# hahnec/stofnet

Measured on AMD Instinct MI355X. Metric: RF waveforms/sec StofNet inference rf_scale=10, higher is better.
Workload: dtype f32 via split-fp16 x3 MFMA operands (hi+lo, fp32 accumulate), device-side exact-f32 re-run on fp16 range overflow; 1 GPU; C2 StofNet.forward [4096,1,2000] -> [4096,1,20000] per GPU, upsample_factor=10, SemiGlobalBlock on, seeded-random weights (seed 3008); rows_per_gpu=4096, L=2000, upsample_factor=10, precision=auto

## Files before the change

stofnet_amd/csrc/convstack.hip:

```cpp
#include <hip/hip_runtime.h>
#include <stdlib.h>
#include <type_traits>
#include "stof_common.h"
#include "stof_hip_util.h"

namespace stof {
int launch_conv_cl(const float* x, const float* w, const float* bias, const float* residual, const float* saved, float* y,
                   int64_t N, int64_t L, int32_t cin, int32_t cout, int32_t K, int32_t act, int32_t precision,
                   int32_t period, int32_t valid_len, hipStream_t stream, const int* run_if);
}

using namespace stof;

typedef float floatx16 __attribute__((ext_vector_type(16)));
typedef _Float16 half8 __attribute__((ext_vector_type(8)));
typedef _Float16 half4 __attribute__((ext_vector_type(4)));

namespace {

constexpr int LAG_LAST = 34;
constexpr int SGB_NW = 2;
constexpr int SGB_WAVES_PER_SIMD = (SGB_NW <= 2) ? 2 : 1;
constexpr int ROWB = ROWF * 4;

// ... 868 lines not shown
                else tail(std::false_type{});
                STAMP_ADD(5);
                __syncthreads();
                STAMP_ADD(2);
                continue;
            }
            auto last_chunks = [&]() {
#pragma unroll
                for (int cc = 0; cc < BODY_CHUNKS_LAST; cc += 2) { do_chunk(wf[0], bf0, bf1, cc); do_chunk(wf[1], bf1, bf0, cc + 1); }
            };
            last_chunks();
            STAMP_ADD(4);

            {
                bool valid[NT];
                int tt[NT], nn[NT];
#pragma unroll
                for (int k = 0; k < NT; ++k) {
                    const int off = 32 * (NT * ni + k) + ln;
                    const int g = R0 + off;
                    decode_row(nR, tR, off, nn[k], tt[k]);
                    int nw, tw;
                    vmap(n0 + nn[k], tt[k], nw, tw);
                    valid[k] = (g >= 0) && (g < gend) && (tt[k] < L) && (tw >= 0) && (tw < Ltrue) &&
                               (tt[k] >= p.halo) && (tt[k] < p.halo + p.seg_len);
                    nn[k] = nw - n0;
                    tt[k] = tw;
                }
                if (p.status != nullptr) {
                    bool bad = false;
#pragma unroll
                    for (int k = 0; k < NT; ++k)
#pragma unroll
                        for (int e = 0; e < 16; ++e) bad = bad || !(fabsf(acc[k][e]) <= 3.0e38f);
                    if (__any(bad) && lane == 0) atomicOr(p.status, 1);
                }
#pragma unroll
                for (int k = 0; k < NT; ++k) {
                    if (!valid[k]) continue;
                    float* const orow = p.y + ((size_t)(n0 + nn[k]) * Ltrue + tt[k]) * r;
#pragma unroll
                    for (int gg = 0; gg < 4; ++gg) {
                        const int c0 = 32 * mi + 8 * gg + 4 * lh;
                        if (c0 >= r) continue;
                        const float vv[4] = {acc[k][4 * gg], acc[k][4 * gg + 1], acc[k][4 * gg + 2], acc[k][4 * gg + 3]};
                        if ((r & 3) == 0) {
                            st4(orow + c0, make_float4(vv[0], vv[1], vv[2], vv[3]));
                        } else {
#pragma unroll
                            for (int e = 0; e < 4; ++e)
                                if (c0 + e < r) orow[c0 + e] = vv[e];
                        }
                    }
                }
            }
            STAMP_ADD(5);
            __syncthreads();
            STAMP_ADD(2);
            }
        }
    }
#ifdef STOF_STAMPS
    if (lane == 0 && p.stamps) {
        unsigned long long* o = p.stamps + ((size_t)blockIdx.x * 4 + wave) * 8;
        for (int i = 0; i < 6; ++i) o[i] = tsum[i];
        o[6] = stamp() - tstart;
        o[7] = (unsigned long long)nsteps;
    }
#endif
}

constexpr int BODY_P2_C1F = 640;
#include "body_p2.h"

struct SgbParams {
    const float* x;
    float* pooled;
    const float* c1;
    const float* cbias;
    const float* chunks;
    int N, L, P, tiles_per_wf;
    const int* run_if;
    unsigned char* arg;
};

template <int PREC, int NW, bool ARG = false>
__global__ __launch_bounds__(256, SGB_WAVES_PER_SIMD) void sgb_contract_pool_kernel(const SgbParams p) {
    constexpr int SHAPE = PREC == STOF_PREC_F16X3 ? 16 : 32;
    static_assert(!ARG || PREC == STOF_PREC_F16X3, "the arg-max output lives in the split-fp16 form");
    static_assert(NW % 2 == 0, "80*NW must be a multiple of 32");
    constexpr int ROWS = SGB_SCALE * NW;
    constexpr int MT = ROWS / 32;
    constexpr int TR = ROWS + 4;
    constexpr int RAWN = TR + 8;
    constexpr int RF = SHAPE == 16 ? ROWF16 : ROWF;
    constexpr int ROWB = RF * 4;
    extern __shared__ __attribute__((aligned(16))) float smem[];
    char* const act = reinterpret_cast<char*>(smem);
    float* const raw = smem + TR * RF;

    const int tid = threadIdx.x;
    const int lane = tid & 63, wave = tid >> 6;
    const int ln = lane & 31, lh = lane >> 5;
    const int n = blockIdx.x / p.tiles_per_wf;
    const int w0 = (blockIdx.x - n * p.tiles_per_wf) * NW;
    const int L = p.L;
    const int tbase = SGB_SCALE * w0 - 2;
    if (p.run_if != nullptr && *p.run_if == 0) return;

    const uint4* const wbase = reinterpret_cast<const uint4*>(p.chunks) + wave * 64 + lane;
    auto wload = [&](int c, int f) -> uint4 { return wbase[((size_t)c * FRAGS_PER_CHUNK + f) * 256]; };
    uint4 wf[2][FRAGS_PER_CHUNK];
#pragma unroll
    for (int f = 0; f < FRAGS_PER_CHUNK; ++f) {
        wf[0][f] = wload(0, f);
        wf[1][f] = wload(1, f);
    }

    for (int i = tid; i < RAWN; i += 256) {
        const int t = tbase - 4 + i;
        raw[i] = (t >= 0 && t < L) ? p.x[(size_t)n * L + t] : 0.f;
    }
    __syncthreads();
    {
        const int cq = tid & 15, rl = tid >> 4;
        float w1[4][9], b1[4];
#pragma unroll
        for (int i = 0; i < 4; ++i) {
#pragma unroll
            for (int d = 0; d < 9; ++d) w1[i][d] = p.c1[(4 * cq + i) * 10 + d];
            b1[i] = p.c1[(4 * cq + i) * 10 + 9];
        }
        for (int row = rl; row < TR; row += 16) {
            const int t = tbase + row;
            float v[4];
#pragma unroll
            for (int i = 0; i < 4; ++i) {
                float a = b1[i];
#pragma unroll
                for (int d = 0; d < 9; ++d) a = fmaf(w1[i][d], raw[row + d], a);
                v[i] = fmaxf(a, 0.f);
            }
            const bool valid = (t >= 0) && (t < L);
            store_act4<PREC>(act + row * ROWB, 4 * cq,
                             valid ? make_float4(v[0], v[1], v[2], v[3]) : make_float4(0.f, 0.f, 0.f, 0.f));
        }
    }
    __syncthreads();

    int c = 0;
    if constexpr (SHAPE == 16) {
        constexpr int MW = SGB_SCALE / 16;
        const int j16 = lane & 15, q4 = lane >> 4;
        for (int ocb = 0; ocb < 4; ++ocb) {
            floatx4 acc[NW][MW][2];
#pragma unroll
            for (int w = 0; w < NW; ++w)
#pragma unroll
                for (int m = 0; m < MW; ++m)
#pragma unroll
                    for (int nt = 0; nt < 2; ++nt)
#pragma unroll
                        for (int e = 0; e < 4; ++e) acc[w][m][nt][e] = 0.f;
            constexpr int NUNIT = 10 * NW;
            auto aload = [&](uint4 (&a)[MW][2], int uu) {
                const int cc = uu / NW, w = uu % NW;
                const int d = cc >> 1, hh = cc & 1;
                const char* arow = act + (SGB_SCALE * w + j16 + d) * ROWB + 64 * hh + 16 * q4;
#pragma unroll
                for (int m = 0; m < MW; ++m) {
                    a[m][0] = ldq(arow + 16 * m * ROWB);
                    a[m][1] = ldq(arow + 16 * m * ROWB + 128);
                }
            };
            auto mfma16 = [](const uint4& a, const uint4& b, floatx4 cacc) {
                return __builtin_amdgcn_mfma_f32_16x16x32_f16(as_h8(a), as_h8(b), cacc, 0, 0, 0);
            };
            auto do_unit = [&](uint4 (&acur)[MW][2], uint4 (&anext)[MW][2], int uu) {
                const int cc = uu / NW, w = uu % NW;
                uint4 (&wq)[FRAGS_PER_CHUNK] = wf[cc & 1];
                const int c2 = (c + 2 < SGB_NCHUNK) ? c + 2 : 0;
                aload(anext, uu + 1 < NUNIT ? uu + 1 : 0);
#pragma unroll
                for (int m = 0; m < MW; ++m) {
                    acc[w][m][0] = mfma16(acur[m][0], wq[0], acc[w][m][0]);
                    acc[w][m][1] = mfma16(acur[m][0], wq[2], acc[w][m][1]);
                    acc[w][m][0] = mfma16(acur[m][1], wq[0], acc[w][m][0]);
                    acc[w][m][1] = mfma16(acur[m][1], wq[2], acc[w][m][1]);
                    acc[w][m][0] = mfma16(acur[m][0], wq[1], acc[w][m][0]);
                    acc[w][m][1] = mfma16(acur[m][0], wq[3], acc[w][m][1]);
                }
                if (w == NW - 1) {
#pragma unroll
                    for (int f = 0; f < FRAGS_PER_CHUNK; ++f) wq[f] = wload(c2, f);
                    ++c;
                }
#pragma unroll
                for (int i = 0; i < MW * 2; ++i) {
                    __builtin_amdgcn_sched_group_barrier(0x008, 3, 0);
                    __builtin_amdgcn_sched_group_barrier(0x100, 1, 0);
                }
                if (w == NW - 1) __builtin_amdgcn_sched_group_barrier(0x020, FRAGS_PER_CHUNK, 0);
                __builtin_amdgcn_sched_barrier(0);
            };
            uint4 af0[MW][2], af1[MW][2];
            if (ocb == 0) aload(af0, 0);
            static_assert(NUNIT % 2 == 0, "units alternate between two fragment sets");
#pragma unroll
            for (int uu = 0; uu < NUNIT; uu += 2) {
                do_unit(af0, af1, uu);
                do_unit(af1, af0, uu + 1);
            }
#pragma unroll
            for (int nt = 0; nt < 2; ++nt) {
                const int oc = 128 * ocb + 32 * wave + 16 * nt + j16;
                const float bias = p.cbias[oc];
#pragma unroll
                for (int w = 0; w < NW; ++w) {
                    float mval = -INFINITY;
                    if constexpr (ARG) {
                        int bi = 0;
#pragma unroll
                        for (int m = 0; m < MW; ++m)
#pragma unroll
                            for (int e = 0; e < 4; ++e) {
                                const float v = acc[w][m][nt][e];
                                const bool up = v > mval;
                                mval = up ? v : mval;
                                bi = up ? 16 * m + 4 * q4 + e : bi;
                            }
#pragma unroll
                        for (int off = 16; off <= 32; off <<= 1) {
                            const float ov = __shfl_xor(mval, off);
                            const int oi = __shfl_xor(bi, off);
                            const bool take = (ov > mval) || (ov == mval && oi < bi);
                            mval = take ? ov : mval;
                            bi = take ? oi : bi;
                        }
                        if (q4 == 0 && w0 + w < p.P) p.arg[((size_t)n * p.P + w0 + w) * NF_SGB + oc] = (unsigned char)bi;
                    } else {
#pragma unroll
                        for (int m = 0; m < MW; ++m)
#pragma unroll
                            for (int e = 0; e < 4; ++e) mval = fmaxf(mval, acc[w][m][nt][e]);
                        mval = fmaxf(mval, __shfl_xor(mval, 16));
                        mval = fmaxf(mval, __shfl_xor(mval, 32));
                    }
                    mval += bias;
                    mval = mval > 0.f ? mval : 0.01f * mval;
                    if (q4 == 0 && w0 + w < p.P)
                        p.pooled[((size_t)n * p.P + w0 + w) * NF_SGB + oc] = mval;
                }
            }
        }
    } else {
    for (int ocb = 0; ocb < 4; ++ocb) {
        floatx16 acc[MT];
#pragma unroll
        for (int m = 0; m < MT; ++m)
#pragma unroll
            for (int e = 0; e < 16; ++e) acc[m][e] = 0.f;

        constexpr int UPC = FRAGS_PER_CHUNK;
        constexpr int NUNIT = 10 * UPC;
        auto aload = [&](uint4 (&a)[MT], int uu) {
            const int cc = uu / UPC, sub = uu % UPC;
            const int d = cc >> 1, hh = cc & 1;
            const char* arow = act + (ln + d) * ROWB;
#pragma unroll
            for (int m = 0; m < MT; ++m) a[m] = ldq(arow + 32 * m * ROWB + act_frag_off(sub, hh, lh));
        };
        auto do_unit = [&](uint4 (&acur)[MT], uint4 (&anext)[MT], int uu) {
            const int cc = uu / UPC, sub = uu % UPC;
            uint4 (&w)[FRAGS_PER_CHUNK] = wf[cc & 1];
            const int c2 = (c + 2 < SGB_NCHUNK) ? c + 2 : 0;
            aload(anext, uu + 1 < NUNIT ? uu + 1 : 0);
#pragma unroll
            for (int m = 0; m < MT; ++m) acc[m] = mma_fp32(acur[m], w[sub], acc[m]);
            w[sub] = wload(c2, sub);
#pragma unroll
            for (int i = 0; i < MT; ++i) {
                __builtin_amdgcn_sched_group_barrier(0x008, 4, 0);
                __builtin_amdgcn_sched_group_barrier(0x100, 1, 0);
            }
            if (sub == UPC - 1) ++c;
            __builtin_amdgcn_sched_barrier(0);
        };
        uint4 af0[MT], af1[MT];
        if (ocb == 0) aload(af0, 0);
#pragma unroll
        for (int uu = 0; uu < NUNIT; uu += 2) {
            do_unit(af0, af1, uu);
            do_unit(af1, af0, uu + 1);
        }
        const int oc = 128 * ocb + 32 * wave + ln;
        const float bias = p.cbias[oc];
        float wmax[NW];
#pragma unroll
        for (int w = 0; w < NW; ++w) wmax[w] = -INFINITY;
#pragma unroll
        for (int m = 0; m < MT; ++m)
#pragma unroll
            for (int v = 0; v < 16; ++v) {
                const int w = (32 * m + 8 * (v >> 2)) / SGB_SCALE;
                wmax[w] = fmaxf(wmax[w], acc[m][v]);
            }
#pragma unroll
        for (int w = 0; w < NW; ++w) {
            float mval = fmaxf(wmax[w], __shfl_xor(wmax[w], 32));
            mval += bias;
            mval = mval > 0.f ? mval : 0.01f * mval;
            if (lh == 0 && w0 + w < p.P)
                p.pooled[((size_t)n * p.P + w0 + w) * NF_SGB + oc] = mval;
        }
    }
    }
}

__global__ __launch_bounds__(256) void onsets_finalize_kernel(const OnsetPartial* __restrict__ ws, int nslots, int nb, int r,
                                                              int half, int* __restrict__ counts, int* __restrict__ idx,
                                                              long long idx_cap) {
    const int lane = threadIdx.x & 63;
    const int row = blockIdx.x * 4 + (threadIdx.x >> 6);
    if (row >= nb) return;
    const OnsetPartial* e = ws + (size_t)row * nslots;
    float m = -INFINITY, lo = INFINITY;
    for (int s = lane; s < nslots; s += 64)
        if (e[s].written) { m = fmaxf(m, e[s].m); lo = fminf(lo, e[s].lo); }
#pragma unroll
    for (int o = 32; o > 0; o >>= 1) { m = fmaxf(m, __shfl_xor(m, o)); lo = fminf(lo, __shfl_xor(lo, o)); }
    const bool emit = (m > 0.f) || (m < 0.f && (lo == m || half == 0));
    int nout = 0;
    if (emit) {
        const unsigned long long lt_mask = (lane == 0) ? 0ull : (~0ull >> (64 - lane));
        int* out = idx + (long long)row * idx_cap;
        for (int s0 = 0; s0 < nslots; s0 += 64) {
            const int sl = s0 + lane;
            unsigned long long match = __ballot(sl < nslots && e[sl].written && e[sl].m == m);
            while (match) {
            const int s = s0 + __builtin_ctzll(match);
            match &= match - 1;
            const OnsetPartial p = e[s];
            for (int q0 = 0; q0 < 16 * r; q0 += 64) {
                const int q = q0 + lane, j = q / r, c = q - j * r;
                const bool hit = q < 16 * r && ((p.eq[c & 3] >> (j + 16 * (c >> 2))) & 1ull);
                const unsigned long long hm = __ballot(hit);
                if (hit) {
                    const long long pos = nout + __builtin_popcountll(hm & lt_mask);
                    if (pos < idx_cap) out[pos] = (p.tw_base + j) * r + c;
                }
                nout += __builtin_popcountll(hm);
            }
            }
        }
    }
    if (lane == 0) counts[row] = nout;
}

constexpr int BODY_S = 192, BODY_RING = 256, BODY_RAWRING = 256;
inline bool body_p2_rows_ok(int seg_len, int halo) { return seg_len + 2 * halo + GAP >= 2 * BODY_S; }
constexpr int ONSET_MAX_SEGS = 32;

constexpr int64_t onset_seg_slots(int64_t seg_len) { return seg_len / 16 + 2; }
constexpr int64_t onset_max_slots(int64_t L) { return L / 16 + 3 * ONSET_MAX_SEGS; }

struct OnsetArgs {
    OnsetPartial* ws;
    int32_t* counts;
    int32_t* idx;
    int64_t idx_cap;
    int half;
};
constexpr int64_t SUB_BATCH = 4096;

constexpr size_t sgb_lds_bytes(int rowf) {
    return (size_t)((SGB_SCALE * SGB_NW + 4) * rowf + SGB_SCALE * SGB_NW + 12) * sizeof(float);
}

template <int PREC>
int launch_forward(const stof_net_desc* desc, const void* packed_dev, const float* x, float* y, int64_t N,
                   int64_t L, void* workspace, hipStream_t stream, void* const* events, int32_t* status,
                   const int32_t* run_if, const OnsetArgs* onsets = nullptr) {
    const int force_nseg_log2 = desc->seg_policy > 0 ? desc->seg_policy - 1 : -1;
    const int r = desc->upsample_factor;
    const bool has_sgb = desc->semi_global_scale != 1;
    const int64_t P = L / SGB_SCALE;
    const int64_t rem = L - P * SGB_SCALE;

    const float* base = static_cast<const float*>(packed_dev);
    uint64_t off = sizeof(PackedHeader) / sizeof(float);
    const float* c1 = base + off;      off += 64 * 10;
    const float* bias = base + off;    off += 13 * 64;
    const float* body = base + off;    off += (uint64_t)BODY_NCHUNK * BODY_CHUNK_F;
    const float* last16 = nullptr;
    if (PREC == STOF_PREC_F16X3 && r <= 16) { last16 = base + off; off += LAST16_F; }
    const float* cbias = base + off;   off += NF_SGB;
    const float* cchunks = base + off; off += (uint64_t)SGB_NCHUNK * SGB_CHUNK_F;
    const float* ew = base + off;      off += 5ull * NF_SGB * NF;
    const float* ebias = base + off;

    static const bool body_p2 = PREC == STOF_PREC_F16X3 && body_p2_enabled();
    constexpr int RF = PREC == STOF_PREC_F16X3 ? ROWF16 : ROWF;
    using Lds = BodyLds<BODY_S, BODY_RING, BODY_RAWRING, RF>;
    const size_t body_p2_bytes = Lds::BYTES + BODY_P2_C1F * sizeof(float);
    const auto body_kernel = &body_sweep_kernel<PREC, BODY_S, BODY_RING, BODY_RAWRING>;
    const auto body_p2_kernel = &body_sweep_p2_kernel<BODY_S, BODY_RING, BODY_RAWRING>;
    const auto sgb_kernel = &sgb_contract_pool_kernel<PREC, SGB_NW>;
    const size_t sgb_bytes = sgb_lds_bytes(RF);
    static LdsLimitOnce body_lds, body_p2_lds, sgb_lds;
    if (int st = body_lds.ensure(reinterpret_cast<const void*>(body_kernel), (int)Lds::BYTES)) return st;
    if (body_p2)
        if (int st = body_p2_lds.ensure(reinterpret_cast<const void*>(body_p2_kernel), (int)body_p2_bytes)) return st;
    if (int st = sgb_lds.ensure(reinterpret_cast<const void*>(sgb_kernel), (int)sgb_bytes)) return st;
    const int ncu = device_cu_count();

    for (int64_t b0 = 0; b0 < N; b0 += SUB_BATCH) {
        const int64_t nb = (N - b0) < SUB_BATCH ? (N - b0) : SUB_BATCH;
        const float* xb = x + b0 * L;
        float* yb = y ? y + b0 * L * r : nullptr;
        float* pooled = nullptr;
        float* sgb = nullptr;
        const bool ev = events && b0 == 0;
        if (ev) (void)hipEventRecord(static_cast<hipEvent_t>(events[0]), stream);
        if (has_sgb && P > 0) {
            pooled = static_cast<float*>(workspace);
            sgb = pooled + nb * P * NF_SGB;
            SgbParams sp;
            sp.x = xb; sp.pooled = pooled; sp.c1 = c1; sp.cbias = cbias; sp.chunks = cchunks;
            sp.N = (int)nb; sp.L = (int)L; sp.P = (int)P;
            sp.tiles_per_wf = (int)((P + SGB_NW - 1) / SGB_NW);
            sp.run_if = run_if;
            sp.arg = nullptr;
            hipLaunchKernelGGL(sgb_kernel, dim3((unsigned)(nb * sp.tiles_per_wf)), dim3(256), sgb_bytes, stream, sp);
            if (ev) (void)hipEventRecord(static_cast<hipEvent_t>(events[1]), stream);
            {
                const int st = stof::launch_conv_cl(pooled, ew, ebias, nullptr, nullptr, sgb, 1, nb * (P + 2), NF_SGB, NF, 5,
                                                     2, PREC, (int)(P + 2), (int)P, stream, run_if);
                if (st != STOF_OK) return st;
            }
            if (ev) (void)hipEventRecord(static_cast<hipEvent_t>(events[2]), stream);
        } else if (ev) {
            (void)hipEventRecord(static_cast<hipEvent_t>(events[1]), stream);
            (void)hipEventRecord(static_cast<hipEvent_t>(events[2]), stream);
        }
        BodyParams bp;
        bp.x = xb; bp.sgb = (has_sgb && P > 0) ? sgb : nullptr; bp.y = yb;
        bp.c1 = c1; bp.bias = bias; bp.chunks = body; bp.last16 = last16;
        bp.N = (int)nb; bp.L = (int)L; bp.r = r; bp.P = (int)P; bp.rem_half = (int)(rem / 2);
        bp.stamps = nullptr;
        bp.dump = nullptr; bp.dump_stride = 0;
        bp.gin = nullptr; bp.fwd_dump = nullptr;
        bp.status = status;
        bp.run_if = run_if;
        bp.nseg_log2 = 0;
        {
            int64_t best = -1;
            for (int k = 0; k <= 5; ++k) {
                const int64_t ns = (int64_t)1 << k;
                if (k > 0 && L / ns < BODY_S / 2) break;
                const int64_t lv = (L + ns - 1) / ns + (k > 0 ? 76 : 0);
                const int64_t nvk = nb * ns;
                const int64_t w = nvk < ncu ? nvk : ncu;
                const int64_t per = (nvk + w - 1) / w;
                const int64_t steps = (per * (lv + GAP) - GAP + LAG_LAST + BODY_S - 1) / BODY_S;
                if (best < 0 || steps < best) { best = steps; bp.nseg_log2 = k; }
            }
        }
        int64_t nseg = (int64_t)1 << bp.nseg_log2;
        if (force_nseg_log2 >= 0) { bp.nseg_log2 = force_nseg_log2; nseg = (int64_t)1 << force_nseg_log2; }
        bp.seg_len = (int)((L + nseg - 1) / nseg);
        bp.halo = nseg > 1 ? 38 : 0;
        const int64_t nv = nb * nseg;
        bp.N = (int)nv;
        bp.onset_ws = nullptr; bp.onset_slots = 0; bp.onset_seg_slots = 0;
        if (onsets != nullptr) {
            bp.onset_seg_slots = (int)onset_seg_slots(bp.seg_len);
            bp.onset_slots = (int)(nseg * bp.onset_seg_slots);
            bp.onset_ws = onsets->ws;
            if (hipMemsetAsync(onsets->ws, 0, (size_t)nb * bp.onset_slots * sizeof(OnsetPartial), stream) != hipSuccess)
                return STOF_ERR_HIP;
        }
#ifdef STOF_STAMPS
        if (workspace) bp.stamps = reinterpret_cast<unsigned long long*>(static_cast<char*>(workspace) + (size_t)(nb * P * (NF_SGB + NF)) * sizeof(float) + 256);
#endif
        int64_t wgs = nv < ncu ? nv : ncu;
        bp.wf_per_wg = (int)((nv + wgs - 1) / wgs);
        wgs = (nv + bp.wf_per_wg - 1) / bp.wf_per_wg;
        if (body_p2 && body_p2_rows_ok(bp.seg_len, bp.halo))
            hipLaunchKernelGGL(body_p2_kernel, dim3((unsigned)wgs), dim3(256), body_p2_bytes, stream, bp);
        else
            hipLaunchKernelGGL(body_kernel, dim3((unsigned)wgs), dim3(256), Lds::BYTES, stream, bp);
        if (ev) (void)hipEventRecord(static_cast<hipEvent_t>(events[3]), stream);
        if (onsets != nullptr)
            hipLaunchKernelGGL(onsets_finalize_kernel, dim3((unsigned)((nb + 3) / 4)), dim3(256), 0, stream, onsets->ws,
                               bp.onset_slots, (int)nb, r, onsets->half, onsets->counts + b0, onsets->idx + b0 * onsets->idx_cap,
                               (long long)onsets->idx_cap);
    }
    if (hipGetLastError() != hipSuccess) return STOF_ERR_HIP;
    return STOF_OK;
}

int forward_impl(const stof_net_desc* desc, const void* packed_dev, const float* x, float* y, int64_t N, int64_t L,
                 void* workspace, size_t workspace_bytes, void* stream_, void* const* events, int32_t* status,
                 const int32_t* run_if = nullptr, const OnsetArgs* onsets = nullptr) {
    if (!desc || N < 0 || L < 0) return STOF_ERR_BAD_ARG;
    if (desc->precision != STOF_PREC_FP32 && desc->precision != STOF_PREC_F16X3) return STOF_ERR_UNSUPPORTED;
    if (desc->seg_policy < 0 || desc->seg_policy > 6) return STOF_ERR_UNSUPPORTED;
    const int r = desc->upsample_factor;
    if (r < 1 || r > 64) return STOF_ERR_UNSUPPORTED;
    const bool has_sgb = desc->semi_global_scale != 1;
    if (has_sgb && desc->semi_global_scale != SGB_SCALE) return STOF_ERR_UNSUPPORTED;
    const int64_t P = L / SGB_SCALE;
    if (has_sgb && L > 0 && P == 0) return STOF_ERR_POOL_EMPTY;
    if (has_sgb && ((L - P * SGB_SCALE) & 1)) return STOF_ERR_ODD_SGB_REMAINDER;
    if (N == 0 || L == 0) return STOF_OK;
    if (!packed_dev || !x || (!y && !onsets)) return STOF_ERR_BAD_ARG;
    if ((L + GAP) * SUB_BATCH > 0x7fffffffLL) return STOF_ERR_UNSUPPORTED;
    if (has_sgb && (!workspace || workspace_bytes < stof_forward_workspace_bytes(desc, N, L)))
        return STOF_ERR_WORKSPACE;
    hipStream_t stream = static_cast<hipStream_t>(stream_);
    if (desc->precision == STOF_PREC_FP32)
        return launch_forward<STOF_PREC_FP32>(desc, packed_dev, x, y, N, L, workspace, stream, events, status, run_if, onsets);
    return launch_forward<STOF_PREC_F16X3>(desc, packed_dev, x, y, N, L, workspace, stream, events, status, run_if, onsets);
}

}

extern "C" size_t stof_forward_workspace_bytes(const stof_net_desc* desc, int64_t N, int64_t L) {
    if (!desc || N <= 0 || L <= 0 || desc->semi_global_scale == 1) return 0;
    const int64_t nb = N < SUB_BATCH ? N : SUB_BATCH;
    const int64_t P = L / SGB_SCALE;
#ifdef STOF_STAMPS
    return (size_t)(nb * P * (NF_SGB + NF)) * sizeof(float) + 256 + 256 * 4 * 8 * 8 + 64;
#else
    return (size_t)(nb * P * (NF_SGB + NF)) * sizeof(float) + 256;
#endif
}

extern "C" int stof_forward(const stof_net_desc* desc, const void* packed_dev, const float* x, float* y,
                            int64_t N, int64_t L, void* workspace, size_t workspace_bytes, void* stream) {
    return forward_impl(desc, packed_dev, x, y, N, L, workspace, workspace_bytes, stream, nullptr, nullptr);
}

extern "C" int stof_forward_checked(const stof_net_desc* desc, const void* packed_dev, const float* x, float* y,
                                    int64_t N, int64_t L, void* workspace, size_t workspace_bytes, void* stream,
                                    int32_t* status_dev) {
    if (!status_dev) return STOF_ERR_BAD_ARG;
    return forward_impl(desc, packed_dev, x, y, N, L, workspace, workspace_bytes, stream, nullptr, status_dev);
}

extern "C" int stof_forward_events(const stof_net_desc* desc, const void* packed_dev, const float* x, float* y,
                                   int64_t N, int64_t L, void* workspace, size_t workspace_bytes, void* stream,
                                   void* const* events, int32_t* status_dev) {
    if (!events) return STOF_ERR_BAD_ARG;
    for (int e = 0; e < STOF_FORWARD_EVENTS; ++e)
        if (!events[e]) return STOF_ERR_BAD_ARG;
    return forward_impl(desc, packed_dev, x, y, N, L, workspace, workspace_bytes, stream, events, status_dev);
}

static size_t onsets_partials_offset(const stof_net_desc* desc, int64_t N, int64_t L) {
    return (stof_forward_workspace_bytes(desc, N, L) + 255) / 256 * 256;
}

extern "C" size_t stof_forward_onsets_workspace_bytes(const stof_net_desc* desc, int64_t N, int64_t L) {
    if (!desc || N <= 0 || L <= 0) return 0;
    const int64_t nb = N < SUB_BATCH ? N : SUB_BATCH;
    return onsets_partials_offset(desc, N, L) + (size_t)nb * onset_max_slots(L) * sizeof(OnsetPartial);
}

extern "C" int stof_forward_onsets(const stof_net_desc* desc, const void* packed_dev, const float* x, float* y, int64_t N,
                                   int64_t L, int32_t window_size, int32_t* counts, int32_t* idx, int64_t idx_cap,
                                   void* workspace, size_t workspace_bytes, void* stream, int32_t* status_dev) {
    if (!desc || !counts || (!idx && idx_cap > 0) || idx_cap < 0 || window_size < 0) return STOF_ERR_BAD_ARG;
    if (desc->precision != STOF_PREC_F16X3 || desc->upsample_factor > 16 || L < 32)
        return STOF_ERR_UNSUPPORTED;
    if (N > 0 && L > 0 && (!workspace || workspace_bytes < stof_forward_onsets_workspace_bytes(desc, N, L))) return STOF_ERR_WORKSPACE;
    OnsetArgs oa;
    oa.ws = reinterpret_cast<OnsetPartial*>(static_cast<char*>(workspace) + onsets_partials_offset(desc, N, L));
    oa.counts = counts; oa.idx = idx; oa.idx_cap = idx_cap;
    oa.half = (window_size / 2 * 2 + 1 - 1) / 2;
    return forward_impl(desc, packed_dev, x, y, N, L, workspace, workspace_bytes, stream, nullptr, status_dev, nullptr, &oa);
}

extern "C" int stof_forward_auto(const stof_net_desc* desc, const void* packed_f16x3_dev, const void* packed_fp32_dev,
                                 const float* x, float* y, int64_t N, int64_t L, void* workspace, size_t workspace_bytes,
                                 void* stream, int32_t* status_dev, void* const* events) {
    if (!desc || !status_dev) return STOF_ERR_BAD_ARG;
    if (events)
        for (int e = 0; e < STOF_FORWARD_EVENTS; ++e)
            if (!events[e]) return STOF_ERR_BAD_ARG;
    stof_net_desc d16 = *desc, d32 = *desc;
    d16.precision = STOF_PREC_F16X3;
    d32.precision = STOF_PREC_FP32;
    if (N > 0 && L > 0 && hipMemsetAsync(status_dev, 0, sizeof(int32_t), static_cast<hipStream_t>(stream)) != hipSuccess)
        return STOF_ERR_HIP;
    const int st = forward_impl(&d16, packed_f16x3_dev, x, y, N, L, workspace, workspace_bytes, stream, events, status_dev);
    if (st != STOF_OK) return st;
    return forward_impl(&d32, packed_fp32_dev, x, y, N, L, workspace, workspace_bytes, stream, nullptr, nullptr, status_dev);
}

namespace {

struct SweepPackArgs {
    const float* p[26];
    float* blob;
    int r;
};

__global__ __launch_bounds__(256) void sweep_pack_kernel(const SweepPackArgs a) {
    const long long i = blockIdx.x * 256ll + threadIdx.x;
    const long long n_c1 = 640, n_bias = 13 * 64, n_body = (long long)BODY_NCHUNK * BODY_CHUNK_F * 2;
    const long long n_last = a.r <= 16 ? (long long)LAST16_F * 2 : 0;
    if (i < n_c1) {
        const int c = (int)(i / 10), t = (int)(i % 10);
        a.blob[i] = t < 9 ? a.p[0][c * 9 + t] : a.p[1][c];
        return;
    }
    long long k = i - n_c1;
// ... 133 lines not shown
    bp.c1 = base; bp.bias = base + 640; bp.chunks = base + 640 + 13 * 64;
    bp.last16 = r <= 16 ? bp.chunks + (size_t)BODY_NCHUNK * BODY_CHUNK_F : nullptr;
    bp.L = (int)L; bp.r = r; bp.P = (int)P; bp.rem_half = (int)((L - P * SGB_SCALE) / 2);
    bp.stamps = nullptr; bp.status = nullptr; bp.run_if = nullptr;
    bp.onset_ws = nullptr; bp.onset_slots = 0; bp.onset_seg_slots = 0;
    bp.dump = dump; bp.dump_stride = (long long)N * L * NF;
    bp.gin = nullptr; bp.fwd_dump = nullptr;
#ifdef STOF_STAMPS
    bp.stamps = train_stamp_buf(0);
#endif
    int64_t wgs = 0;
    if (int st = train_sweep_geometry(desc, bp, N, L, &wgs)) return st;
    if (p2 && !body_p2_rows_ok(bp.seg_len, bp.halo)) {
        if (split) return STOF_ERR_UNSUPPORTED;
        auto k3 = &body_sweep_kernel<STOF_PREC_F16X3, BODY_S, BODY_RING, BODY_RAWRING, true, false>;
        static LdsLimitOnce lds3;
        if (int st = lds3.ensure(reinterpret_cast<const void*>(k3), (int)Lds16::BYTES)) return st;
        hipLaunchKernelGGL(k3, dim3((unsigned)wgs), dim3(256), Lds16::BYTES, stream, bp);
        return hipGetLastError() == hipSuccess ? STOF_OK : STOF_ERR_HIP;
    }
    hipLaunchKernelGGL(kernel, dim3((unsigned)wgs), dim3(256), lds_bytes, stream, bp);
    return hipGetLastError() == hipSuccess ? STOF_OK : STOF_ERR_HIP;
}

extern "C" int stof_train_sweep(const stof_net_desc* desc, const void* blob_dev, const float* x, const float* sgb_expand,
                                float* dump, float* y, int64_t N, int64_t L, void* stream) {
    return train_sweep_impl(desc, blob_dev, x, sgb_expand, dump, y, N, L, stream, false);
}
extern "C" int stof_train_sweep_split(const stof_net_desc* desc, const void* blob_dev, const float* x, const float* sgb_expand,
                                      float* dump, float* y, int64_t N, int64_t L, void* stream) {
    return train_sweep_impl(desc, blob_dev, x, sgb_expand, dump, y, N, L, stream, true);
}

namespace {
struct SgbPackArgs {
    const float* c1w; const float* c1b; const float* cw; const float* cb;
    float* blob;
};
__global__ __launch_bounds__(256) void sgb_pack_kernel(const SgbPackArgs a) {
    const long long i = blockIdx.x * 256ll + threadIdx.x;
    const long long n_c1 = 640, n_cb = NF_SGB, n_body = (long long)SGB_NCHUNK * SGB_CHUNK_F * 2;
    if (i < n_c1) {
        const int c = (int)(i / 10), t = (int)(i % 10);
        a.blob[i] = t < 9 ? a.c1w[c * 9 + t] : a.c1b[c];
        return;
    }
    long long k = i - n_c1;
    if (k < n_cb) { a.blob[n_c1 + k] = a.cb[k]; return; }
    k -= n_cb;
    if (k >= n_body) return;
    const int e = (int)(k & 7), lane = (int)((k >> 3) & 63), tile = (int)((k >> 9) & 3), frag = (int)((k >> 11) & 3);
    const int c = (int)(k >> 13);
    const int hh = c & 1, tap = (c >> 1) % 5, ocb = c / 10;
    const int nt = frag >> 1, part = frag & 1, j = lane & 15, q = lane >> 4;
    const int o = 128 * ocb + 32 * tile + 16 * nt + j;
    const float v = a.cw[((size_t)o * NF + 32 * hh + 8 * q + e) * 5 + tap];
    const _Float16 hi = (_Float16)v;
    reinterpret_cast<_Float16*>(a.blob + n_c1 + n_cb)[k] = part == 0 ? hi : (_Float16)(v - (float)hi);
}
}

extern "C" size_t stof_train_sgb_blob_bytes(void) { return (640 + NF_SGB + (size_t)SGB_NCHUNK * SGB_CHUNK_F) * sizeof(float); }

extern "C" int stof_train_sgb_contract_pool(const float* conv1_w, const float* conv1_b, const float* contract_w, const float* contract_b,
                                            void* blob_dev, const float* x, float* pooled, uint8_t* arg, int64_t N, int64_t L,
                                            void* stream_) {
    if (N < 0 || L < 0) return STOF_ERR_BAD_ARG;
    const int64_t P = L / SGB_SCALE;
    if (L > 0 && P == 0) return STOF_ERR_POOL_EMPTY;
    if (N == 0 || L == 0) return STOF_OK;
    if (!conv1_w || !conv1_b || !contract_w || !contract_b || !blob_dev || !x || !pooled || !arg) return STOF_ERR_BAD_ARG;
    hipStream_t stream = static_cast<hipStream_t>(stream_);
    SgbPackArgs a;
    a.c1w = conv1_w; a.c1b = conv1_b; a.cw = contract_w; a.cb = contract_b; a.blob = static_cast<float*>(blob_dev);
    const long long total = 640 + NF_SGB + (long long)SGB_NCHUNK * SGB_CHUNK_F * 2;
    hipLaunchKernelGGL(sgb_pack_kernel, dim3((unsigned)((total + 255) / 256)), dim3(256), 0, stream, a);
    auto kernel = &sgb_contract_pool_kernel<STOF_PREC_F16X3, SGB_NW, true>;
    static LdsLimitOnce lds;
    if (int st = lds.ensure(reinterpret_cast<const void*>(kernel), (int)sgb_lds_bytes(ROWF16))) return st;
    SgbParams sp;
    sp.x = x; sp.pooled = pooled; sp.c1 = a.blob; sp.cbias = a.blob + 640; sp.chunks = a.blob + 640 + NF_SGB;
    sp.N = (int)N; sp.L = (int)L; sp.P = (int)P;
    sp.tiles_per_wf = (int)((P + SGB_NW - 1) / SGB_NW);
    sp.run_if = nullptr; sp.arg = arg;
    if (N * sp.tiles_per_wf > 0x7fffffffLL) return STOF_ERR_UNSUPPORTED;
    hipLaunchKernelGGL(kernel, dim3((unsigned)(N * sp.tiles_per_wf)), dim3(256), sgb_lds_bytes(ROWF16), stream, sp);
    return hipGetLastError() == hipSuccess ? STOF_OK : STOF_ERR_HIP;
}

namespace {
struct SweepPackBwdArgs {
    const float* w[11];
    float* blob;
};
__global__ __launch_bounds__(256) void sweep_pack_bwd_kernel(const SweepPackBwdArgs a) {
    const long long i = blockIdx.x * 256ll + threadIdx.x;
    const long long n_head = 640 + 13 * 64, n_body = (long long)BODY_NCHUNK * BODY_CHUNK_F * 2;
    if (i < n_head) { a.blob[i] = 0.f; return; }
    const long long k = i - n_head;
    if (k >= n_body) return;
    _Float16* const body = reinterpret_cast<_Float16*>(a.blob + n_head);
    const int e = (int)(k & 7), lane = (int)((k >> 3) & 63), blk = (int)((k >> 9) & 1), frag = (int)((k >> 10) & 3);
    const int c = (int)(k >> 12);
    if (c >= 11 * BODY_CHUNKS_K7) { body[k] = (_Float16)0.f; return; }
    const int j = 1 + c / BODY_CHUNKS_K7, cc = c % BODY_CHUNKS_K7;
    const int tap = cc >> 1, hh = cc & 1, m = frag >> 1, part = frag & 1, i16 = lane & 15, q = lane >> 4;
    const int arow = body16_out_channel(blk, m, i16);
    const int b = 32 * hh + 8 * q + e;
    const float v = a.w[11 - j][((size_t)b * NF + arow) * 7 + (6 - tap)];
    const _Float16 hi = (_Float16)v;
    body[k] = part == 0 ? hi : (_Float16)(v - (float)hi);
}
}

extern "C" int stof_train_sweep_bwd_pack(const float* const* conv_weights_dev, void* blob_dev, void* stream) {
    if (!conv_weights_dev || !blob_dev) return STOF_ERR_BAD_ARG;
    SweepPackBwdArgs a;
    for (int i = 0; i < 11; ++i) {
        if (!conv_weights_dev[i]) return STOF_ERR_BAD_ARG;
        a.w[i] = conv_weights_dev[i];
    }
    a.blob = static_cast<float*>(blob_dev);
    const long long total = 640 + 13 * 64 + (long long)BODY_NCHUNK * BODY_CHUNK_F * 2;
    hipLaunchKernelGGL(sweep_pack_bwd_kernel, dim3((unsigned)((total + 255) / 256)), dim3(256), 0, static_cast<hipStream_t>(stream), a);
    return hipGetLastError() == hipSuccess ? STOF_OK : STOF_ERR_HIP;
}

static int train_sweep_bwd_impl(const stof_net_desc* desc, const void* blob_dev, const float* g6, const float* fwd_dump,
                                float* dump, int64_t N, int64_t L, void* stream_, bool split) {
    if (!desc || N < 0 || L < 0) return STOF_ERR_BAD_ARG;
    if (N == 0 || L == 0) return STOF_OK;
    if (!blob_dev || !g6 || !fwd_dump || !dump) return STOF_ERR_BAD_ARG;
    if ((L + GAP) * N > 0x7fffffffLL || N * L * NF > 0x7fffffffffLL) return STOF_ERR_UNSUPPORTED;
    hipStream_t stream = static_cast<hipStream_t>(stream_);
    using Lds16 = BodyLds<BODY_S, BODY_RING, BODY_RAWRING, ROWF16>;
    static const bool p2 = body_p2_enabled();
    if (split && !p2) return STOF_ERR_UNSUPPORTED;
    auto kernel = split ? &body_sweep_p2_kernel<BODY_S, BODY_RING, BODY_RAWRING, true, true, true>
                  : p2  ? &body_sweep_p2_kernel<BODY_S, BODY_RING, BODY_RAWRING, true, true>
                        : &body_sweep_kernel<STOF_PREC_F16X3, BODY_S, BODY_RING, BODY_RAWRING, true, true>;
    const size_t lds_bytes = Lds16::BYTES + (p2 ? BODY_P2_C1F * sizeof(float) : 0);
    static LdsLimitOnce lds[2];
    if (int st = lds[split ? 1 : 0].ensure(reinterpret_cast<const void*>(kernel), (int)lds_bytes)) return st;
    const float* base = static_cast<const float*>(blob_dev);
    BodyParams bp;
    bp.x = nullptr; bp.sgb = nullptr; bp.y = nullptr;
    bp.c1 = base; bp.bias = base + 640; bp.chunks = base + 640 + 13 * 64; bp.last16 = nullptr;
    bp.L = (int)L; bp.r = 1; bp.P = 0; bp.rem_half = 0;
    bp.stamps = nullptr; bp.status = nullptr; bp.run_if = nullptr;
    bp.onset_ws = nullptr; bp.onset_slots = 0; bp.onset_seg_slots = 0;
    bp.dump = dump; bp.dump_stride = (long long)N * L * NF;
    bp.gin = g6; bp.fwd_dump = fwd_dump;
#ifdef STOF_STAMPS
    bp.stamps = train_stamp_buf(1);
#endif
    int64_t wgs = 0;
    if (int st = train_sweep_geometry(desc, bp, N, L, &wgs)) return st;
    if (p2 && !body_p2_rows_ok(bp.seg_len, bp.halo)) {
        if (split) return STOF_ERR_UNSUPPORTED;
        auto k3 = &body_sweep_kernel<STOF_PREC_F16X3, BODY_S, BODY_RING, BODY_RAWRING, true, true>;
        static LdsLimitOnce lds3;
        if (int st = lds3.ensure(reinterpret_cast<const void*>(k3), (int)Lds16::BYTES)) return st;
        hipLaunchKernelGGL(k3, dim3((unsigned)wgs), dim3(256), Lds16::BYTES, stream, bp);
        return hipGetLastError() == hipSuccess ? STOF_OK : STOF_ERR_HIP;
    }
    hipLaunchKernelGGL(kernel, dim3((unsigned)wgs), dim3(256), lds_bytes, stream, bp);
    return hipGetLastError() == hipSuccess ? STOF_OK : STOF_ERR_HIP;
// ... 34 lines not shown
```

Measured before the change: 255,100 waveforms/s.

## Screen max-pool candidates with hi-only MFMA pass and Cauchy-Schwarz bounds

The split-fp16 SemiGlobalBlock contraction now first computes only the hi×hi product. It then uses per-row activation norms and per-channel weight norms (Cauchy-Schwarz) to bound the omitted lo terms. Rows whose upper bound cannot beat the best lower bound are dropped, and the full three-term product is recomputed only for the surviving candidate rows, grouped into 16-row MFMA tiles. This aims to cut the MFMA work of the pooled contraction, at the cost of extra LDS, a small weight-norm kernel, list building with DPP/readlane, and branchy recompute paths.

```diff
diff --git a/stofnet_amd/csrc/convstack.hip b/stofnet_amd/csrc/convstack.hip
--- a/stofnet_amd/csrc/convstack.hip
+++ b/stofnet_amd/csrc/convstack.hip
@@ -974,7 +974,13 @@
     int N, L, P, tiles_per_wf;
     const int* run_if;
     unsigned char* arg;
+    const float* wnorm;
 };
+
+constexpr int SGB_SCREEN_RSQ_F = 2 * (SGB_SCALE * SGB_NW + 4);
+constexpr int SGB_SCREEN_NRM_F = 2 * SGB_SCALE * SGB_NW;
+constexpr int SGB_SCREEN_LIST_B = 4 * 2 * SGB_NW * SGB_SCALE;
+constexpr int SGB_RING = 5;
 
 template <int PREC, int NW, bool ARG = false>
 __global__ __launch_bounds__(256, SGB_WAVES_PER_SIMD) void sgb_contract_pool_kernel(const SgbParams p) {
@@ -987,9 +993,13 @@
     constexpr int RAWN = TR + 8;
     constexpr int RF = SHAPE == 16 ? ROWF16 : ROWF;
     constexpr int ROWB = RF * 4;
+    constexpr bool SCREEN = SHAPE == 16 && !ARG;
+    static_assert(!SCREEN || (TR * RF + RAWN) % 4 == 0, "the screening arrays are read 16 bytes at a time");
     extern __shared__ __attribute__((aligned(16))) float smem[];
     char* const act = reinterpret_cast<char*>(smem);
     float* const raw = smem + TR * RF;
+    float* const rsq = raw + RAWN;
+    float* const nrm = rsq + SGB_SCREEN_RSQ_F;
 
     const int tid = threadIdx.x;
     const int lane = tid & 63, wave = tid >> 6;
@@ -1002,11 +1012,13 @@
 
     const uint4* const wbase = reinterpret_cast<const uint4*>(p.chunks) + wave * 64 + lane;
     auto wload = [&](int c, int f) -> uint4 { return wbase[((size_t)c * FRAGS_PER_CHUNK + f) * 256]; };
-    uint4 wf[2][FRAGS_PER_CHUNK];
-#pragma unroll
-    for (int f = 0; f < FRAGS_PER_CHUNK; ++f) {
-        wf[0][f] = wload(0, f);
-        wf[1][f] = wload(1, f);
+    constexpr int WFN = SCREEN ? 2 : FRAGS_PER_CHUNK;
+    constexpr int WFS = SCREEN ? 2 : 1;
+    uint4 wf[2][WFN];
+#pragma unroll
+    for (int f = 0; f < WFN; ++f) {
+        wf[0][f] = wload(0, WFS * f);
+        wf[1][f] = wload(1, WFS * f);
     }
 
     for (int i = tid; i < RAWN; i += 256) {
@@ -1036,12 +1048,253 @@
             const bool valid = (t >= 0) && (t < L);
             store_act4<PREC>(act + row * ROWB, 4 * cq,
                              valid ? make_float4(v[0], v[1], v[2], v[3]) : make_float4(0.f, 0.f, 0.f, 0.f));
+            if constexpr (SCREEN) {
+                float sh = 0.f, sl = 0.f;
+#pragma unroll
+                for (int i = 0; i < 4; ++i) {
+                    const float u = valid ? v[i] : 0.f;
+                    const float hf = (float)(_Float16)u;
+                    const float lf = (float)(_Float16)(u - hf);
+                    sh = fmaf(hf, hf, sh);
+                    sl = fmaf(lf, lf, sl);
+                }
+#pragma unroll
+                for (int off = 1; off < 16; off <<= 1) {
+                    sh += __shfl_xor(sh, off);
+                    sl += __shfl_xor(sl, off);
+                }
+                if (cq == 0) {
+                    rsq[2 * row] = sh;
+                    rsq[2 * row + 1] = sl;
+                }
+            }
         }
     }
     __syncthreads();
+    if constexpr (SCREEN) {
+        if (tid < ROWS) {
+            float sh = 0.f, sl = 0.f;
+#pragma unroll
+            for (int d = 0; d < 5; ++d) {
+                sh += rsq[2 * (tid + d)];
+                sl += rsq[2 * (tid + d) + 1];
+            }
+            nrm[2 * tid] = sqrtf(sh) * (1.f + 0x1p-16f);
+            nrm[2 * tid + 1] = sqrtf(sl) * (1.f + 0x1p-16f);
+        }
+        __syncthreads();
+    }
 
     int c = 0;
-    if constexpr (SHAPE == 16) {
+    if constexpr (SCREEN) {
+        constexpr int MW = SGB_SCALE / 16;
+        const int j16 = lane & 15, q4 = lane >> 4;
+        unsigned char* const lists = reinterpret_cast<unsigned char*>(nrm + SGB_SCREEN_NRM_F) + wave * (2 * NW * SGB_SCALE);
+        auto mfma16 = [](const uint4& a, const uint4& b, floatx4 cacc) {
+            return __builtin_amdgcn_mfma_f32_16x16x32_f16(as_h8(a), as_h8(b), cacc, 0, 0, 0);
+        };
+        for (int ocb = 0; ocb < 4; ++ocb) {
+            floatx4 acc[NW][MW][2];
+#pragma unroll
+            for (int w = 0; w < NW; ++w)
+#pragma unroll
+                for (int m = 0; m < MW; ++m)
+#pragma unroll
+                    for (int nt = 0; nt < 2; ++nt)
+#pragma unroll
+                        for (int e = 0; e < 4; ++e) acc[w][m][nt][e] = 0.f;
+            constexpr int NUNIT = 10 * NW;
+            auto aload = [&](uint4 (&a)[MW], int uu) {
+                const int cc = uu / NW, w = uu % NW;
+                const int d = cc >> 1, hh = cc & 1;
+                const char* arow = act + (SGB_SCALE * w + j16 + d) * ROWB + 64 * hh + 16 * q4;
+#pragma unroll
+                for (int m = 0; m < MW; ++m) a[m] = ldq(arow + 16 * m * ROWB);
+            };
+            auto do_unit = [&](uint4 (&acur)[MW], uint4 (&anext)[MW], int uu) {
+                const int cc = uu / NW, w = uu % NW;
+                uint4 (&wq)[2] = wf[cc & 1];
+                const int c2 = (c + 2 < SGB_NCHUNK) ? c + 2 : 0;
+                if (uu + 1 < NUNIT) aload(anext, uu + 1);
+#pragma unroll
+                for (int m = 0; m < MW; ++m) {
+                    acc[w][m][0] = mfma16(acur[m], wq[0], acc[w][m][0]);
+                    acc[w][m][1] = mfma16(acur[m], wq[1], acc[w][m][1]);
+                }
+                if (w == NW - 1) {
+                    wq[0] = wload(c2, 0);
+                    wq[1] = wload(c2, 2);
+                    ++c;
+                }
+#pragma unroll
+                for (int i = 0; i < MW; ++i) {
+                    __builtin_amdgcn_sched_group_barrier(0x008, 2, 0);
+                    __builtin_amdgcn_sched_group_barrier(0x100, 1, 0);
+                }
+                if (w == NW - 1) __builtin_amdgcn_sched_group_barrier(0x020, 2, 0);
+                __builtin_amdgcn_sched_barrier(0);
+            };
+            uint4 af0[MW], af1[MW];
+            aload(af0, 0);
+            static_assert(NUNIT % 2 == 0, "units alternate between two fragment sets");
+#pragma unroll
+            for (int uu = 0; uu < NUNIT; uu += 2) {
+                do_unit(af0, af1, uu);
+                do_unit(af1, af0, uu + 1);
+            }
+
+            const int cb = 10 * ocb;
+            uint4 wr[SGB_RING][2];
+#pragma unroll
+            for (int k = 0; k < SGB_RING; ++k) {
+                wr[k][0] = wload(cb + k, 0);
+                wr[k][1] = wload(cb + k, 1);
+            }
+
+            int gsel[2];
+#pragma unroll
+            for (int nt = 0; nt < 2; ++nt) {
+                const int oc = 128 * ocb + 32 * wave + 16 * nt + j16;
+                const float nwh = p.wnorm[oc], nwl = p.wnorm[NF_SGB + oc];
+                const float k1 = fmaf(0x1p-12f, nwh, nwl);
+                int gmax = 1;
+#pragma unroll
+                for (int w = 0; w < NW; ++w) {
+                    float s[MW][4];
+                    float low = -INFINITY;
+                    bool bad = false;
+#pragma unroll
+                    for (int m = 0; m < MW; ++m) {
+                        const float4* np = reinterpret_cast<const float4*>(nrm + 2 * (SGB_SCALE * w + 16 * m + 4 * q4));
+                        const float4 n01 = np[0], n23 = np[1];
+                        const float nah[4] = {n01.x, n01.z, n23.x, n23.z}, nal[4] = {n01.y, n01.w, n23.y, n23.w};
+#pragma unroll
+                        for (int e = 0; e < 4; ++e) {
+                            const float B = fmaf(nah[e], k1, nal[e] * nwh) * (1.f + 0x1p-10f);
+                            const float hh = acc[w][m][nt][e];
+                            const float dlo = hh - B;
+                            s[m][e] = hh + B;
+                            bad |= !(fabsf(dlo) < INFINITY) || !(fabsf(s[m][e]) < INFINITY);
+                            low = fmaxf(low, dlo);
+                        }
+                    }
+                    low = fmaxf(low, __shfl_xor(low, 16));
+                    low = fmaxf(low, __shfl_xor(low, 32));
+                    unsigned mask = 0;
+#pragma unroll
+                    for (int m = 0; m < MW; ++m)
+#pragma unroll
+                        for (int e = 0; e < 4; ++e) mask |= (s[m][e] < low ? 0u : 1u) << (4 * m + e);
+                    if (__any(bad)) mask = 0xFFFFFu;
+                    if (w0 + w >= p.P) mask = q4 == 0 ? 1u : 0u;
+                    mask |= (unsigned)__builtin_amdgcn_update_dpp(0, (int)mask, 0x121, 0xF, 0xF, false);
+                    mask |= (unsigned)__builtin_amdgcn_update_dpp(0, (int)mask, 0x122, 0xF, 0xF, false);
+                    mask |= (unsigned)__builtin_amdgcn_update_dpp(0, (int)mask, 0x124, 0xF, 0xF, false);
+                    mask |= (unsigned)__builtin_amdgcn_update_dpp(0, (int)mask, 0x128, 0xF, 0xF, false);
+                    unsigned mq[4];
+#pragma unroll
+                    for (int q = 0; q < 4; ++q) mq[q] = (unsigned)__builtin_amdgcn_readlane((int)mask, 16 * q);
+                    if ((mq[0] | mq[1] | mq[2] | mq[3]) == 0) {
+                        mask = 0xFFFFFu;
+                        mq[0] = mq[1] = mq[2] = mq[3] = 0xFFFFFu;
+                    }
+                    const int c0 = __builtin_popcount(mq[0]), c1 = __builtin_popcount(mq[1]), c2 = __builtin_popcount(mq[2]);
+                    const int ncand = c0 + c1 + c2 + __builtin_popcount(mq[3]);
+                    const int g = (ncand + 15) >> 4;
+                    gmax = g > gmax ? g : gmax;
+                    const int fq = mq[0] ? 0 : mq[1] ? 1 : mq[2] ? 2 : 3;
+                    const int fb = __builtin_ctz(mq[fq]);
+                    const int padrow = 16 * (fb >> 2) + 4 * fq + (fb & 3);
+                    unsigned char* const lst = lists + (nt * NW + w) * SGB_SCALE;
+                    lst[lane] = (unsigned char)padrow;
+                    if (lane < SGB_SCALE - 64) lst[64 + lane] = (unsigned char)padrow;
+                    __builtin_amdgcn_fence(__ATOMIC_RELEASE, "wavefront");
+                    __builtin_amdgcn_wave_barrier();
+                    const int pre = (q4 > 0 ? c0 : 0) + (q4 > 1 ? c1 : 0) + (q4 > 2 ? c2 : 0);
+#pragma unroll
+                    for (int pass = 0; pass < 2; ++pass) {
+                        const int b = j16 + 16 * pass;
+                        if (b < 4 * MW && ((mask >> b) & 1u))
+                            lst[pre + __builtin_popcount(mask & ((1u << b) - 1u))] = (unsigned char)(16 * (b >> 2) + 4 * q4 + (b & 3));
+                    }
+                }
+                gsel[nt] = gmax;
+            }
+            __builtin_amdgcn_fence(__ATOMIC_ACQ_REL, "wavefront");
+            __builtin_amdgcn_wave_barrier();
+
+            auto recompute = [&](auto GC, const int nt) {
+                constexpr int G = decltype(GC)::value;
+                int roff[NW][G];
+                floatx4 r[NW][G];
+#pragma unroll
+                for (int w = 0; w < NW; ++w)
+#pragma unroll
+                    for (int g = 0; g < G; ++g) {
+                        roff[w][g] = (SGB_SCALE * w + lists[(nt * NW + w) * SGB_SCALE + 16 * g + j16]) * ROWB + 16 * q4;
+#pragma unroll
+                        for (int e = 0; e < 4; ++e) r[w][g][e] = 0.f;
+                    }
+#pragma unroll
+                for (int cc = 0; cc < 10; ++cc) {
+                    const int d = cc >> 1, hh = cc & 1;
+                    uint4 (&wq)[2] = wr[cc % SGB_RING];
+                    uint4 a[NW][G][2];
+#pragma unroll
+                    for (int w = 0; w < NW; ++w)
+#pragma unroll
+                        for (int g = 0; g < G; ++g) {
+                            const char* arow = act + roff[w][g] + d * ROWB + 64 * hh;
+                            a[w][g][0] = ldq(arow);
+                            a[w][g][1] = ldq(arow + 128);
+                        }
+#pragma unroll
+                    for (int w = 0; w < NW; ++w)
+#pragma unroll
+                        for (int g = 0; g < G; ++g) r[w][g] = mfma16(a[w][g][0], wq[0], r[w][g]);
+#pragma unroll
+                    for (int w = 0; w < NW; ++w)
+#pragma unroll
+                        for (int g = 0; g < G; ++g) r[w][g] = mfma16(a[w][g][1], wq[0], r[w][g]);
+#pragma unroll
+                    for (int w = 0; w < NW; ++w)
+#pragma unroll
+                        for (int g = 0; g < G; ++g) r[w][g] = mfma16(a[w][g][0], wq[1], r[w][g]);
+                    static_assert(10 % SGB_RING == 0, "the ring phase is the same at the start of every N-tile");
+                    if (cc + SGB_RING < 10) {
+                        wq[0] = wload(cb + cc + SGB_RING, 2 * nt);
+                        wq[1] = wload(cb + cc + SGB_RING, 2 * nt + 1);
+                    } else if (nt == 0) {
+                        wq[0] = wload(cb + cc + SGB_RING - 10, 2);
+                        wq[1] = wload(cb + cc + SGB_RING - 10, 3);
+                    }
+                }
+                const int oc = 128 * ocb + 32 * wave + 16 * nt + j16;
+                const float bias = p.cbias[oc];
+#pragma unroll
+                for (int w = 0; w < NW; ++w) {
+                    float mval = -INFINITY;
+#pragma unroll
+                    for (int g = 0; g < G; ++g)
+#pragma unroll
+                        for (int e = 0; e < 4; ++e) mval = fmaxf(mval, r[w][g][e]);
+                    mval = fmaxf(mval, __shfl_xor(mval, 16));
+                    mval = fmaxf(mval, __shfl_xor(mval, 32));
+                    mval += bias;
+                    mval = mval > 0.f ? mval : 0.01f * mval;
+                    if (q4 == 0 && w0 + w < p.P)
+                        p.pooled[((size_t)n * p.P + w0 + w) * NF_SGB + oc] = mval;
+                }
+            };
+#pragma unroll 1
+            for (int nt = 0; nt < 2; ++nt) {
+                const int g = nt == 0 ? gsel[0] : gsel[1];
+                if (g == 1) recompute(std::integral_constant<int, 1>{}, nt);
+                else if (g == 2) recompute(std::integral_constant<int, 2>{}, nt);
+                else recompute(std::integral_constant<int, MW>{}, nt);
+            }
+        }
+    } else if constexpr (SHAPE == 16) {
         constexpr int MW = SGB_SCALE / 16;
         const int j16 = lane & 15, q4 = lane >> 4;
         for (int ocb = 0; ocb < 4; ++ocb) {
@@ -1110,34 +1363,26 @@
 #pragma unroll
                 for (int w = 0; w < NW; ++w) {
                     float mval = -INFINITY;
-                    if constexpr (ARG) {
-                        int bi = 0;
-#pragma unroll
-                        for (int m = 0; m < MW; ++m)
-#pragma unroll
-                            for (int e = 0; e < 4; ++e) {
-                                const float v = acc[w][m][nt][e];
-                                const bool up = v > mval;
-                                mval = up ? v : mval;
-                                bi = up ? 16 * m + 4 * q4 + e : bi;
-                            }
-#pragma unroll
-                        for (int off = 16; off <= 32; off <<= 1) {
-                            const float ov = __shfl_xor(mval, off);
-                            const int oi = __shfl_xor(bi, off);
-                            const bool take = (ov > mval) || (ov == mval && oi < bi);
-                            mval = take ? ov : mval;
-                            bi = take ? oi : bi;
+                    static_assert(ARG, "split-fp16 inference runs the screened form above");
+                    int bi = 0;
+#pragma unroll
+                    for (int m = 0; m < MW; ++m)
+#pragma unroll
+                        for (int e = 0; e < 4; ++e) {
+                            const float v = acc[w][m][nt][e];
+                            const bool up = v > mval;
+                            mval = up ? v : mval;
+                            bi = up ? 16 * m + 4 * q4 + e : bi;
                         }
-                        if (q4 == 0 && w0 + w < p.P) p.arg[((size_t)n * p.P + w0 + w) * NF_SGB + oc] = (unsigned char)bi;
-                    } else {
-#pragma unroll
-                        for (int m = 0; m < MW; ++m)
-#pragma unroll
-                            for (int e = 0; e < 4; ++e) mval = fmaxf(mval, acc[w][m][nt][e]);
-                        mval = fmaxf(mval, __shfl_xor(mval, 16));
-                        mval = fmaxf(mval, __shfl_xor(mval, 32));
+#pragma unroll
+                    for (int off = 16; off <= 32; off <<= 1) {
+                        const float ov = __shfl_xor(mval, off);
+                        const int oi = __shfl_xor(bi, off);
+                        const bool take = (ov > mval) || (ov == mval && oi < bi);
+                        mval = take ? ov : mval;
+                        bi = take ? oi : bi;
                     }
+                    if (q4 == 0 && w0 + w < p.P) p.arg[((size_t)n * p.P + w0 + w) * NF_SGB + oc] = (unsigned char)bi;
                     mval += bias;
                     mval = mval > 0.f ? mval : 0.01f * mval;
                     if (q4 == 0 && w0 + w < p.P)
@@ -1265,8 +1510,40 @@
 };
 constexpr int64_t SUB_BATCH = 4096;
 
-constexpr size_t sgb_lds_bytes(int rowf) {
-    return (size_t)((SGB_SCALE * SGB_NW + 4) * rowf + SGB_SCALE * SGB_NW + 12) * sizeof(float);
+constexpr size_t sgb_lds_bytes(int rowf, bool screen = false) {
+    return (size_t)((SGB_SCALE * SGB_NW + 4) * rowf + SGB_SCALE * SGB_NW + 12 + (screen ? SGB_SCREEN_RSQ_F + SGB_SCREEN_NRM_F : 0)) *
+               sizeof(float) + (screen ? SGB_SCREEN_LIST_B : 0);
+}
+constexpr size_t SGB_WNORM_BYTES = 2 * NF_SGB * sizeof(float);
+
+__global__ __launch_bounds__(256) void sgb_weight_norms_kernel(const float* __restrict__ chunks, float* __restrict__ wnorm,
+                                                               const int* run_if) {
+    if (run_if != nullptr && *run_if == 0) return;
+    const int ocb = blockIdx.x >> 1, nt = blockIdx.x & 1, tid = threadIdx.x;
+    const uint4* const base = reinterpret_cast<const uint4*>(chunks) + tid;
+    float sq[2] = {0.f, 0.f};
+    for (int cc = 0; cc < 10; ++cc)
+#pragma unroll
+        for (int part = 0; part < 2; ++part) {
+            const half8 h = as_h8(base[((size_t)(10 * ocb + cc) * FRAGS_PER_CHUNK + 2 * nt + part) * 256]);
+#pragma unroll
+            for (int e = 0; e < 8; ++e) sq[part] = fmaf((float)h[e], (float)h[e], sq[part]);
+        }
+#pragma unroll
+    for (int part = 0; part < 2; ++part) {
+        sq[part] += __shfl_xor(sq[part], 16);
+        sq[part] += __shfl_xor(sq[part], 32);
+    }
+    if ((tid & 63) < 16) {
+        const int oc = 128 * ocb + 32 * (tid >> 6) + 16 * nt + (tid & 15);
+        wnorm[oc] = sqrtf(sq[0]) * (1.f + 0x1p-16f);
+        wnorm[NF_SGB + oc] = sqrtf(sq[1]) * (1.f + 0x1p-16f);
+    }
+}
+
+size_t sgb_maps_bytes(int64_t N, int64_t L) {
+    const int64_t nb = N < SUB_BATCH ? N : SUB_BATCH;
+    return (size_t)(nb * (L / SGB_SCALE) * (NF_SGB + NF)) * sizeof(float) + 256;
 }
 
 template <int PREC>
@@ -1298,7 +1575,7 @@
     const auto body_kernel = &body_sweep_kernel<PREC, BODY_S, BODY_RING, BODY_RAWRING>;
     const auto body_p2_kernel = &body_sweep_p2_kernel<BODY_S, BODY_RING, BODY_RAWRING>;
     const auto sgb_kernel = &sgb_contract_pool_kernel<PREC, SGB_NW>;
-    const size_t sgb_bytes = sgb_lds_bytes(RF);
+    const size_t sgb_bytes = sgb_lds_bytes(RF, PREC == STOF_PREC_F16X3);
     static LdsLimitOnce body_lds, body_p2_lds, sgb_lds;
     if (int st = body_lds.ensure(reinterpret_cast<const void*>(body_kernel), (int)Lds::BYTES)) return st;
     if (body_p2)
@@ -1323,6 +1600,13 @@
             sp.tiles_per_wf = (int)((P + SGB_NW - 1) / SGB_NW);
             sp.run_if = run_if;
             sp.arg = nullptr;
+            sp.wnorm = nullptr;
+            if (PREC == STOF_PREC_F16X3) {
+                float* wnorm = reinterpret_cast<float*>(static_cast<char*>(workspace) + sgb_maps_bytes(N, L));
+                if (b0 == 0)
+                    hipLaunchKernelGGL(sgb_weight_norms_kernel, dim3(8), dim3(256), 0, stream, cchunks, wnorm, run_if);
+                sp.wnorm = wnorm;
+            }
             hipLaunchKernelGGL(sgb_kernel, dim3((unsigned)(nb * sp.tiles_per_wf)), dim3(256), sgb_bytes, stream, sp);
             if (ev) (void)hipEventRecord(static_cast<hipEvent_t>(events[1]), stream);
             {
@@ -1373,7 +1657,7 @@
                 return STOF_ERR_HIP;
         }
 #ifdef STOF_STAMPS
-        if (workspace) bp.stamps = reinterpret_cast<unsigned long long*>(static_cast<char*>(workspace) + (size_t)(nb * P * (NF_SGB + NF)) * sizeof(float) + 256);
+        if (workspace) bp.stamps = reinterpret_cast<unsigned long long*>(static_cast<char*>(workspace) + sgb_maps_bytes(N, L) + SGB_WNORM_BYTES);
 #endif
         int64_t wgs = nv < ncu ? nv : ncu;
         bp.wf_per_wg = (int)((nv + wgs - 1) / wgs);
@@ -1420,12 +1704,10 @@
 
 extern "C" size_t stof_forward_workspace_bytes(const stof_net_desc* desc, int64_t N, int64_t L) {
     if (!desc || N <= 0 || L <= 0 || desc->semi_global_scale == 1) return 0;
-    const int64_t nb = N < SUB_BATCH ? N : SUB_BATCH;
-    const int64_t P = L / SGB_SCALE;
 #ifdef STOF_STAMPS
-    return (size_t)(nb * P * (NF_SGB + NF)) * sizeof(float) + 256 + 256 * 4 * 8 * 8 + 64;
+    return sgb_maps_bytes(N, L) + SGB_WNORM_BYTES + 256 * 4 * 8 * 8 + 64;
 #else
-    return (size_t)(nb * P * (NF_SGB + NF)) * sizeof(float) + 256;
+    return sgb_maps_bytes(N, L) + SGB_WNORM_BYTES;
 #endif
 }
 
@@ -1725,7 +2007,7 @@
     sp.x = x; sp.pooled = pooled; sp.c1 = a.blob; sp.cbias = a.blob + 640; sp.chunks = a.blob + 640 + NF_SGB;
     sp.N = (int)N; sp.L = (int)L; sp.P = (int)P;
     sp.tiles_per_wf = (int)((P + SGB_NW - 1) / SGB_NW);
-    sp.run_if = nullptr; sp.arg = arg;
+    sp.run_if = nullptr; sp.arg = arg; sp.wnorm = nullptr;
     if (N * sp.tiles_per_wf > 0x7fffffffLL) return STOF_ERR_UNSUPPORTED;
     hipLaunchKernelGGL(kernel, dim3((unsigned)(N * sp.tiles_per_wf)), dim3(256), sgb_lds_bytes(ROWF16), stream, sp);
     return hipGetLastError() == hipSuccess ? STOF_OK : STOF_ERR_HIP;
```

After: 240,200 waveforms/s. -5.8%, worse.
